# benfred/implicit

Hardware: AMD Instinct MI355X
Metric: ALS user+item updates/sec per iteration (factors=128); top-k recs/sec (higher is better)
Workload: dtype f32; 1 GPU; BASELINE configs[2]: last.fm-360K-shaped synthetic CSR, ALS CG cg_steps=3; users=358868, items=292385, nnz=17308340, factors=128, solver=cg, cg_steps=3

## Files before the change

implicit_amd/csrc/gramian.hip:

```cpp
#include <hip/hip_fp16.h>

#include <type_traits>

#include "common.h"

namespace imp {

typedef float f32x16 __attribute__((ext_vector_type(16)));

namespace {
constexpr int kMaxPairsPerWave = 3;

template <int NV, typename T>
__device__ __forceinline__ void gramian_wave(const T *__restrict__ Y, long n_rows, int f, long r_begin, long r_end,
                                             const int (&ti)[kMaxPairsPerWave], const int (&tj)[kMaxPairsPerWave],
                                             const int (&pair)[kMaxPairsPerWave], int n_pairs, float *__restrict__ out, int lane) {
  const int khalf = lane >> 5;
  f32x16 acc[NV];
#pragma unroll
  for (int t = 0; t < NV; ++t)
#pragma unroll
    for (int e = 0; e < 16; ++e) acc[t][e] = 0.f;
  int ca[NV], cb[NV], mask_a[NV], mask_b[NV];
#pragma unroll
  for (int t = 0; t < NV; ++t) {
    const int c0 = 32 * ti[t] + (lane & 31), c1 = 32 * tj[t] + (lane & 31);
    mask_a[t] = -(int)(c0 < f), mask_b[t] = -(int)(c1 < f);
    ca[t] = min(c0, f - 1), cb[t] = min(c1, f - 1);
  }
  float a[2][4][NV], b[2][4][NV];
  int mask_r[2][4];
  auto fetch = [&](int buf, long r0) {
#pragma unroll
    for (int s = 0; s < 4; ++s) {
      const long r = r0 + 2 * s + khalf;
      mask_r[buf][s] = -(int)(r < r_end);
      const T *row = Y + min(r, n_rows - 1) * (long)f;
#pragma unroll
      for (int t = 0; t < NV; ++t) {
        a[buf][s][t] = (float)row[ca[t]];
        b[buf][s][t] = (float)row[cb[t]];
      }
    }
  };
  auto masked = [](float v, int m) { return __int_as_float(__float_as_int(v) & m); };
  auto multiply = [&](int buf) {
#pragma unroll
    for (int s = 0; s < 4; ++s)
#pragma unroll
      for (int t = 0; t < NV; ++t)
        acc[t] = __builtin_amdgcn_mfma_f32_32x32x2f32(masked(a[buf][s][t], mask_r[buf][s] & mask_a[t]),
                                                      masked(b[buf][s][t], mask_r[buf][s] & mask_b[t]), acc[t], 0, 0, 0);
  };
  fetch(0, r_begin);
  for (long r0 = r_begin; r0 < r_end; r0 += 16) {
    fetch(1, r0 + 8);
    __builtin_amdgcn_sched_barrier(0);
    multiply(0);
    __builtin_amdgcn_sched_barrier(0);
    fetch(0, r0 + 16);
    __builtin_amdgcn_sched_barrier(0);
    multiply(1);
    __builtin_amdgcn_sched_barrier(0);
  }
#pragma unroll
  for (int t = 0; t < NV; ++t) {
    float *tile = out + ((size_t)pair[t]) * 1024;
    (void)n_pairs;
#pragma unroll
    for (int e = 0; e < 16; ++e) {
      const int rr = (e & 3) + 8 * (e >> 2) + 4 * (lane >> 5);
      tile[rr * 32 + (lane & 31)] = acc[t][e];
    }
  }
}
}

template <int TPW, typename T>
__global__ __launch_bounds__(256) void gramian_partial_kernel(const T *__restrict__ Y, long n_rows, int f,
                                                              long rows_per_chunk, float *__restrict__ ws) {
  static_assert(TPW <= kMaxPairsPerWave, "pairs per wave");
  const int lane = threadIdx.x & 63;
  const int wave = __builtin_amdgcn_readfirstlane((int)(threadIdx.x >> 6));
  const int n_tiles = (f + 31) / 32, n_pairs = n_tiles * (n_tiles + 1) / 2;
  const int wrot = (wave + 2 * (int)((blockIdx.x ^ (blockIdx.x >> 8)) & 1)) & 3;
  int ti[kMaxPairsPerWave] = {0, 0, 0}, tj[kMaxPairsPerWave] = {0, 0, 0}, pair[kMaxPairsPerWave] = {0, 0, 0};
  int nv = 0;
#pragma unroll
  for (int s = 0; s < TPW; ++s) {
    const int p = ((int)blockIdx.y * TPW + s) * 4 + wrot;
    if (p < n_pairs) {
      int row = 0, left = p;
      while (left >= n_tiles - row) left -= n_tiles - row, ++row;
      ti[s] = row, tj[s] = row + left, pair[s] = p;
      nv = s + 1;
    }
  }
  const long r_begin = (long)blockIdx.x * rows_per_chunk;
  const long r_end = min(n_rows, r_begin + rows_per_chunk);
  float *out = ws + (size_t)blockIdx.x * n_pairs * 1024;
  if (nv == 3) {
    if constexpr (TPW >= 3) gramian_wave<3, T>(Y, n_rows, f, r_begin, r_end, ti, tj, pair, n_pairs, out, lane);
  } else if (nv == 2) {
    if constexpr (TPW >= 2) gramian_wave<2, T>(Y, n_rows, f, r_begin, r_end, ti, tj, pair, n_pairs, out, lane);
  } else if (nv == 1) {
    gramian_wave<1, T>(Y, n_rows, f, r_begin, r_end, ti, tj, pair, n_pairs, out, lane);
  }
}

template <int N, int I = 0, typename Fn> __device__ __forceinline__ void static_for(Fn &&fn) {
  if constexpr (I < N) {
    fn(std::integral_constant<int, I>{});
    static_for<N, I + 1>(fn);
  }
}
constexpr int tri_row(int n, int p) { int row = 0; while (p >= n - row) p -= n - row, ++row; return row; }
constexpr int tri_col(int n, int p) { int row = 0; while (p >= n - row) p -= n - row, ++row; return row + p; }

template <typename T, int VW> struct FactorVec;
template <> struct FactorVec<float, 4> { using type = float4; };
template <> struct FactorVec<float, 2> { using type = float2; };
template <> struct FactorVec<__half, 4> { using type = uint2; };
template <> struct FactorVec<__half, 2> { using type = unsigned; };

template <int VW> __device__ __forceinline__ void unpack(const float4 &v, float (&o)[VW]) { o[0] = v.x, o[1] = v.y, o[2] = v.z, o[3] = v.w; }
template <int VW> __device__ __forceinline__ void unpack(const float2 &v, float (&o)[VW]) { o[0] = v.x, o[1] = v.y; }
template <int VW> __device__ __forceinline__ void unpack(const uint2 &v, float (&o)[VW]) {
  const float2 a = __half22float2(*reinterpret_cast<const __half2 *>(&v.x)), b = __half22float2(*reinterpret_cast<const __half2 *>(&v.y));
  o[0] = a.x, o[1] = a.y, o[2] = b.x, o[3] = b.y;
}
template <int VW> __device__ __forceinline__ void unpack(const unsigned &v, float (&o)[VW]) {
  const float2 a = __half22float2(*reinterpret_cast<const __half2 *>(&v));
  o[0] = a.x, o[1] = a.y;
}

template <int VW, int WROT, typename T>
__device__ __forceinline__ void gramian_wave_vec(const T *__restrict__ Y, long n_rows, long r_begin, long r_end,
                                                 float *__restrict__ out, int lane) {
  constexpr int F = 32 * VW, NP = VW * (VW + 1) / 2, NV = (NP - WROT + 3) / 4;
  using Vec = typename FactorVec<T, VW>::type;
  if constexpr (NV > 0) {
    const int khalf = lane >> 5;
    f32x16 acc[NV];
#pragma unroll
    for (int t = 0; t < NV; ++t)
#pragma unroll
      for (int e = 0; e < 16; ++e) acc[t][e] = 0.f;
    Vec v[3][4];
    const unsigned off_even = (unsigned)(VW * (lane & 31) * sizeof(T));
    const unsigned off_pair = off_even + (unsigned)(khalf * F * sizeof(T));
    auto fetch = [&](int buf, long r0) {
#pragma unroll
      for (int s = 0; s < 4; ++s) {
        const long rb = min(r0 + 2 * s, n_rows - 1);
        const unsigned off = rb + 1 < n_rows ? off_pair : off_even;
        v[buf][s] = *reinterpret_cast<const Vec *>(reinterpret_cast<const char *>(Y + rb * (long)F) + off);
      }
    };
    auto multiply = [&](auto tail_tag, int buf, long r0) {
      constexpr bool TAIL = decltype(tail_tag)::value;
#pragma unroll
      for (int s = 0; s < 4; ++s) {
        float o[VW];
        unpack<VW>(v[buf][s], o);
        if constexpr (TAIL) {
          const int m = -(int)(r0 + 2 * s + khalf < r_end);
#pragma unroll
          for (int c = 0; c < VW; ++c) o[c] = __int_as_float(__float_as_int(o[c]) & m);
        }
        static_for<NV>([&](auto tc) {
          constexpr int t = decltype(tc)::value, ci = tri_row(VW, WROT + 4 * t), cj = tri_col(VW, WROT + 4 * t);
          acc[t] = __builtin_amdgcn_mfma_f32_32x32x2f32(o[ci], o[cj], acc[t], 0, 0, 0);
        });
      }
    };
    fetch(0, r_begin);
    fetch(1, r_begin + 8);
    long r0 = r_begin;
    for (; r0 + 24 <= r_end; r0 += 24) {
      fetch(2, r0 + 16);
      __builtin_amdgcn_sched_barrier(0);
      multiply(std::false_type{}, 0, r0);
      __builtin_amdgcn_sched_barrier(0);
      fetch(0, r0 + 24);
      __builtin_amdgcn_sched_barrier(0);
      multiply(std::false_type{}, 1, r0 + 8);
      __builtin_amdgcn_sched_barrier(0);
      fetch(1, r0 + 32);
      __builtin_amdgcn_sched_barrier(0);
      multiply(std::false_type{}, 2, r0 + 16);
      __builtin_amdgcn_sched_barrier(0);
    }
    if (r0 < r_end) {
      fetch(2, r0 + 16);
      multiply(std::true_type{}, 0, r0);
      multiply(std::true_type{}, 1, r0 + 8);
      multiply(std::true_type{}, 2, r0 + 16);
    }
#pragma unroll
    for (int t = 0; t < NV; ++t) {
      float *tile = out + (size_t)(WROT + 4 * t) * 1024;
#pragma unroll
      for (int e = 0; e < 16; ++e) {
        const int rr = (e & 3) + 8 * (e >> 2) + 4 * (lane >> 5);
        tile[rr * 32 + (lane & 31)] = acc[t][e];
      }
    }
  }
}

template <int VW, typename T>
__global__ __launch_bounds__(256) void gramian_partial_vec_kernel(const T *__restrict__ Y, long n_rows, long rows_per_chunk,
                                                                  float *__restrict__ ws) {
  constexpr int NP = VW * (VW + 1) / 2;
  const int lane = threadIdx.x & 63;
  const int wave = __builtin_amdgcn_readfirstlane((int)(threadIdx.x >> 6));
  const int wrot = (wave + 2 * (int)((blockIdx.x ^ (blockIdx.x >> 8)) & 1)) & 3;
  const long r_begin = (long)blockIdx.x * rows_per_chunk;
  const long r_end = min(n_rows, r_begin + rows_per_chunk);
  float *out = ws + (size_t)blockIdx.x * NP * 1024;
  if (wrot == 0) gramian_wave_vec<VW, 0, T>(Y, n_rows, r_begin, r_end, out, lane);
  else if (wrot == 1) gramian_wave_vec<VW, 1, T>(Y, n_rows, r_begin, r_end, out, lane);
  else if (wrot == 2) gramian_wave_vec<VW, 2, T>(Y, n_rows, r_begin, r_end, out, lane);
  else gramian_wave_vec<VW, 3, T>(Y, n_rows, r_begin, r_end, out, lane);
}



__global__ __launch_bounds__(1024) void gramian_reduce_kernel(const float *__restrict__ ws, int chunks, int f, float reg,
                                                              float *__restrict__ out, int vw) {
  __shared__ float part[16][64];
  const int n_tiles = vw > 1 ? vw : (f + 31) / 32, n_pairs = n_tiles * (n_tiles + 1) / 2;
  const int e = threadIdx.x & 63, g = threadIdx.x >> 6;
  const int p = blockIdx.x / 16, idx = (blockIdx.x % 16) * 64 + e;
  const size_t stride = (size_t)n_pairs * 1024;
  const float *src = ws + (size_t)p * 1024 + idx;
  float s0 = 0.f, s1 = 0.f, s2 = 0.f, s3 = 0.f;
  int c = g;
  for (; c + 48 < chunks; c += 64) {
    s0 += src[(size_t)c * stride];
    s1 += src[(size_t)(c + 16) * stride];
    s2 += src[(size_t)(c + 32) * stride];
    s3 += src[(size_t)(c + 48) * stride];
  }
  for (; c < chunks; c += 16) s0 += src[(size_t)c * stride];
  part[g][e] = (s0 + s1) + (s2 + s3);
  __syncthreads();
  if (g == 0) {
    float s = 0.f;
#pragma unroll
    for (int k = 0; k < 16; ++k) s += part[k][e];
    int row = 0, left = p;
    while (left >= n_tiles - row) left -= n_tiles - row, ++row;
    const int r = vw > 1 ? vw * (idx / 32) + row : 32 * row + idx / 32;
    const int col = vw > 1 ? vw * (idx & 31) + row + left : 32 * (row + left) + (idx & 31);
    if (r < f && col < f && (left != 0 || r <= col)) {
      if (r == col) s += reg;
      out[(size_t)r * f + col] = s;
      if (r != col) out[(size_t)col * f + r] = s;
    }
  }
}

template <typename T> static void gramian_t(const T *Y, long n_rows, int f, float reg, float *out) {
  const int vw = f == 128 ? 4 : (f == 64 ? 2 : 1);
  const int n_tiles = vw > 1 ? vw : (f + 31) / 32, n_pairs = n_tiles * (n_tiles + 1) / 2;
  const int tpw = std::min(kMaxPairsPerWave, (n_pairs + 3) / 4);
  const int gy = vw > 1 ? 1 : (n_pairs + 4 * tpw - 1) / (4 * tpw);
  long target_chunks = std::max(1, ctx().num_cus * 4 / gy);
  long rows_per_chunk = std::max<long>(256, (n_rows + target_chunks - 1) / target_chunks);
  rows_per_chunk = vw > 1 ? (rows_per_chunk + 23) / 24 * 24 : (rows_per_chunk + 15) / 16 * 16;
  int chunks = n_rows <= 0 ? 0 : (int)std::max<long>(1, (n_rows + rows_per_chunk - 1) / rows_per_chunk);
  size_t need = (size_t)std::max(chunks, 1) * n_pairs * 1024;
  float *ws = ctx().gram_ws.reserve(need);
  if (chunks > 0) {
    IMP_PROF("gramian_partial");
    dim3 grid(chunks, gy, 1);
    if (vw == 4) gramian_partial_vec_kernel<4, T><<<grid, 256, 0, stream()>>>(Y, n_rows, rows_per_chunk, ws);
    else if (vw == 2) gramian_partial_vec_kernel<2, T><<<grid, 256, 0, stream()>>>(Y, n_rows, rows_per_chunk, ws);
    else if (tpw == 1) gramian_partial_kernel<1, T><<<grid, 256, 0, stream()>>>(Y, n_rows, f, rows_per_chunk, ws);
    else if (tpw == 2) gramian_partial_kernel<2, T><<<grid, 256, 0, stream()>>>(Y, n_rows, f, rows_per_chunk, ws);
    else gramian_partial_kernel<3, T><<<grid, 256, 0, stream()>>>(Y, n_rows, f, rows_per_chunk, ws);
    IMP_CHECK_HIP(hipGetLastError());
  }
  {
    IMP_PROF("gramian_reduce");
    gramian_reduce_kernel<<<n_pairs * 16, 1024, 0, stream()>>>(ws, chunks, f, reg, out, vw);
    IMP_CHECK_HIP(hipGetLastError());
  }
}

void gramian(const float *Y, long n_rows, int f, float reg, float *out) { gramian_t<float>(Y, n_rows, f, reg, out); }
void gramian_half(const void *Y, long n_rows, int f, float reg, float *out) {
  gramian_t<__half>(reinterpret_cast<const __half *>(Y), n_rows, f, reg, out);
}

}
```

Measured before the change: 180.4 million updates/s.

## Combine four wave-quads per 1024-thread block and reduce Gramian partials in LDS

Adds a 1024-thread Gramian partial kernel in which four quads of waves each process a row range, and quads 1-3 write their accumulator tiles to LDS. Quad 0 then adds those tiles in and writes a single partial per block. The grid is sized from the occupancy API so it fills every CU. This cuts the number of workspace partials and the global-memory traffic of the later reduce kernel. In exchange it adds a block-wide barrier and a large dynamic LDS allocation (120KB for f=128), which can limit occupancy.

```diff
diff --git a/implicit_amd/csrc/gramian.hip b/implicit_amd/csrc/gramian.hip
--- a/implicit_amd/csrc/gramian.hip
+++ b/implicit_amd/csrc/gramian.hip
@@ -134,18 +134,17 @@
   o[0] = a.x, o[1] = a.y;
 }
 
+template <int VW, int WROT> constexpr int wave_pairs() { return (VW * (VW + 1) / 2 - WROT + 3) / 4; }
+
+__device__ __forceinline__ int tile_slot(int e, int lane) { return ((e & 3) + 8 * (e >> 2) + 4 * (lane >> 5)) * 32 + (lane & 31); }
+
 template <int VW, int WROT, typename T>
-__device__ __forceinline__ void gramian_wave_vec(const T *__restrict__ Y, long n_rows, long r_begin, long r_end,
-                                                 float *__restrict__ out, int lane) {
-  constexpr int F = 32 * VW, NP = VW * (VW + 1) / 2, NV = (NP - WROT + 3) / 4;
+__device__ __forceinline__ void gramian_accumulate_vec(const T *__restrict__ Y, long n_rows, long r_begin, long r_end,
+                                                       f32x16 (&acc)[kMaxPairsPerWave], int lane) {
+  constexpr int F = 32 * VW, NV = wave_pairs<VW, WROT>();
   using Vec = typename FactorVec<T, VW>::type;
   if constexpr (NV > 0) {
     const int khalf = lane >> 5;
-    f32x16 acc[NV];
-#pragma unroll
-    for (int t = 0; t < NV; ++t)
-#pragma unroll
-      for (int e = 0; e < 16; ++e) acc[t][e] = 0.f;
     Vec v[3][4];
     const unsigned off_even = (unsigned)(VW * (lane & 31) * sizeof(T));
     const unsigned off_pair = off_even + (unsigned)(khalf * F * sizeof(T));
@@ -197,16 +196,33 @@
       multiply(std::true_type{}, 1, r0 + 8);
       multiply(std::true_type{}, 2, r0 + 16);
     }
-#pragma unroll
-    for (int t = 0; t < NV; ++t) {
-      float *tile = out + (size_t)(WROT + 4 * t) * 1024;
-#pragma unroll
-      for (int e = 0; e < 16; ++e) {
-        const int rr = (e & 3) + 8 * (e >> 2) + 4 * (lane >> 5);
-        tile[rr * 32 + (lane & 31)] = acc[t][e];
-      }
-    }
-  }
+  }
+}
+
+template <int VW, int WROT> __device__ __forceinline__ void store_tiles(const f32x16 (&acc)[kMaxPairsPerWave], float *out, int lane) {
+#pragma unroll
+  for (int t = 0; t < wave_pairs<VW, WROT>(); ++t)
+#pragma unroll
+    for (int e = 0; e < 16; ++e) out[(WROT + 4 * t) * 1024 + tile_slot(e, lane)] = acc[t][e];
+}
+template <int VW, int WROT> __device__ __forceinline__ void add_tiles(f32x16 (&acc)[kMaxPairsPerWave], const float *in, int lane) {
+#pragma unroll
+  for (int t = 0; t < wave_pairs<VW, WROT>(); ++t)
+#pragma unroll
+    for (int e = 0; e < 16; ++e) acc[t][e] += in[(WROT + 4 * t) * 1024 + tile_slot(e, lane)];
+}
+
+template <typename Fn> __device__ __forceinline__ void with_deal(int wrot, Fn &&fn) {
+  if (wrot == 0) fn(std::integral_constant<int, 0>{});
+  else if (wrot == 1) fn(std::integral_constant<int, 1>{});
+  else if (wrot == 2) fn(std::integral_constant<int, 2>{});
+  else fn(std::integral_constant<int, 3>{});
+}
+__device__ __forceinline__ void clear_tiles(f32x16 (&acc)[kMaxPairsPerWave]) {
+#pragma unroll
+  for (int t = 0; t < kMaxPairsPerWave; ++t)
+#pragma unroll
+    for (int e = 0; e < 16; ++e) acc[t][e] = 0.f;
 }
 
 template <int VW, typename T>
@@ -219,10 +235,40 @@
   const long r_begin = (long)blockIdx.x * rows_per_chunk;
   const long r_end = min(n_rows, r_begin + rows_per_chunk);
   float *out = ws + (size_t)blockIdx.x * NP * 1024;
-  if (wrot == 0) gramian_wave_vec<VW, 0, T>(Y, n_rows, r_begin, r_end, out, lane);
-  else if (wrot == 1) gramian_wave_vec<VW, 1, T>(Y, n_rows, r_begin, r_end, out, lane);
-  else if (wrot == 2) gramian_wave_vec<VW, 2, T>(Y, n_rows, r_begin, r_end, out, lane);
-  else gramian_wave_vec<VW, 3, T>(Y, n_rows, r_begin, r_end, out, lane);
+  f32x16 acc[kMaxPairsPerWave];
+  clear_tiles(acc);
+  with_deal(wrot, [&](auto w) {
+    gramian_accumulate_vec<VW, decltype(w)::value, T>(Y, n_rows, r_begin, r_end, acc, lane);
+    store_tiles<VW, decltype(w)::value>(acc, out, lane);
+  });
+}
+
+template <int VW> constexpr size_t quad_lds_bytes() { return (size_t)3 * (VW * (VW + 1) / 2) * 1024 * sizeof(float); }
+
+template <int VW, typename T>
+__global__ __launch_bounds__(1024) void gramian_quad_vec_kernel(const T *__restrict__ Y, long n_rows, long rows_per_quad,
+                                                                float *__restrict__ ws) {
+  extern __shared__ float quad_sets[];
+  constexpr int NP = VW * (VW + 1) / 2;
+  const int lane = threadIdx.x & 63;
+  const int wave = __builtin_amdgcn_readfirstlane((int)(threadIdx.x >> 6));
+  const int quad = wave >> 2;
+  const int wrot = (wave + 2 * (quad & 1)) & 3;
+  const long r_begin = ((long)blockIdx.x * 4 + quad) * rows_per_quad;
+  const long r_end = min(n_rows, r_begin + rows_per_quad);
+  f32x16 acc[kMaxPairsPerWave];
+  clear_tiles(acc);
+  with_deal(wrot, [&](auto w) {
+    if (r_begin < r_end) gramian_accumulate_vec<VW, decltype(w)::value, T>(Y, n_rows, r_begin, r_end, acc, lane);
+    if (quad != 0) store_tiles<VW, decltype(w)::value>(acc, quad_sets + (size_t)(quad - 1) * NP * 1024, lane);
+  });
+  __syncthreads();
+  if (quad != 0) return;
+  with_deal(wrot, [&](auto w) {
+#pragma unroll 1
+    for (int q = 0; q < 3; ++q) add_tiles<VW, decltype(w)::value>(acc, quad_sets + (size_t)q * NP * 1024, lane);
+    store_tiles<VW, decltype(w)::value>(acc, ws + (size_t)blockIdx.x * NP * 1024, lane);
+  });
 }
 
 
@@ -262,6 +308,20 @@
   }
 }
 
+template <int VW, typename T> static long quad_grid() {
+  static int per_cu[64] = {};
+  constexpr auto kern = gramian_quad_vec_kernel<VW, T>;
+  allow_dynamic_lds_once<kern>(quad_lds_bytes<VW>());
+  const int dev = ctx().device;
+  int n = dev >= 0 && dev < 64 ? per_cu[dev] : 0;
+  if (n == 0) {
+    IMP_CHECK_HIP(hipOccupancyMaxActiveBlocksPerMultiprocessor(&n, reinterpret_cast<const void *>(kern), 1024, quad_lds_bytes<VW>()));
+    if (n < 1) throw std::runtime_error("gramian: the quad kernel does not fit a compute unit");
+    if (dev >= 0 && dev < 64) per_cu[dev] = n;
+  }
+  return (long)ctx().num_cus * n;
+}
+
 template <typename T> static void gramian_t(const T *Y, long n_rows, int f, float reg, float *out) {
   const int vw = f == 128 ? 4 : (f == 64 ? 2 : 1);
   const int n_tiles = vw > 1 ? vw : (f + 31) / 32, n_pairs = n_tiles * (n_tiles + 1) / 2;
@@ -271,9 +331,22 @@
   long rows_per_chunk = std::max<long>(256, (n_rows + target_chunks - 1) / target_chunks);
   rows_per_chunk = vw > 1 ? (rows_per_chunk + 23) / 24 * 24 : (rows_per_chunk + 15) / 16 * 16;
   int chunks = n_rows <= 0 ? 0 : (int)std::max<long>(1, (n_rows + rows_per_chunk - 1) / rows_per_chunk);
+  const bool quads = vw > 1 && n_rows >= 4 * 24;
+  long rows_per_quad = 0;
+  if (quads) {
+    const long wgs = vw == 4 ? quad_grid<4, T>() : quad_grid<2, T>();
+    rows_per_quad = ((n_rows + wgs - 1) / wgs + 3) / 4;
+    rows_per_quad = (rows_per_quad + 23) / 24 * 24;
+    chunks = (int)((n_rows + 4 * rows_per_quad - 1) / (4 * rows_per_quad));
+  }
   size_t need = (size_t)std::max(chunks, 1) * n_pairs * 1024;
   float *ws = ctx().gram_ws.reserve(need);
-  if (chunks > 0) {
+  if (quads) {
+    IMP_PROF("gramian_partial");
+    if (vw == 4) gramian_quad_vec_kernel<4, T><<<chunks, 1024, quad_lds_bytes<4>(), stream()>>>(Y, n_rows, rows_per_quad, ws);
+    else gramian_quad_vec_kernel<2, T><<<chunks, 1024, quad_lds_bytes<2>(), stream()>>>(Y, n_rows, rows_per_quad, ws);
+    IMP_CHECK_HIP(hipGetLastError());
+  } else if (chunks > 0) {
     IMP_PROF("gramian_partial");
     dim3 grid(chunks, gy, 1);
     if (vw == 4) gramian_partial_vec_kernel<4, T><<<grid, 256, 0, stream()>>>(Y, n_rows, rows_per_chunk, ws);
```

Measured after the change: 181.1 million updates/s (median of 6 runs). No clear change (+0.4%).
